# rbuler/multimodal-isic

Measured on AMD Instinct MI355X. Metric: bags/sec (train step) @ 64x224x224 patches/bag, higher is better.
Workload: dtype bf16; 1 GPU; ISIC-shaped attention-MIL: 256 bags x 64x224x224 patches + 128-d radiomics, ResNet-18 encoder, bf16 (BASELINE.json configs[1]); patches_per_bag=64, patch=3x224x224, radiomics_dim=128, parallelism=dp1

## Files before the change

### multimodal-isic_amd/csrc/conv_stem.hip

```cpp
#include <type_traits>

#include "common.h"
#include "slab_sum.inc"
#include "mfma_tile.h"
#include "pool_grad.h"

namespace {

constexpr int TH = 8, TW = 16;
constexpr int PR = 2 * TH + 5, PC = 40;
constexpr int PROW = PC * 8;
constexpr int WROW = 7 * 64 + 16;
constexpr int CPAD = 72;
constexpr int YROW = 128 + 32;
constexpr int STEM_DW_ELEMS = 64 * 7 * 7 * 3;
constexpr int STEM_WGRAD_BLOCKS = 512;
constexpr int STEM_FWD_BLOCKS = 768;

struct StemArgs {
  const unsigned short* in;
  const unsigned short* w;
  unsigned short* out;
  const unsigned short* dy;
  float* dw;
  double* stat_sum;
  double* stat_sumsq;
  int stat_slots;
  int N, Hin, Win, Hout, Wout, tiles_h, tiles_w, total_tiles;
};

constexpr int PATCH_PER_THREAD = (PR * PC + 255) / 256;
__device__ __forceinline__ void fetch_patch(u32x2 (&r)[PATCH_PER_THREAD], const StemArgs& a, int tile, int tid) {
  const int n = tile / (a.tiles_h * a.tiles_w);
  const int t2 = tile - n * (a.tiles_h * a.tiles_w);
  const int oy0 = (t2 / a.tiles_w) * TH, ox0 = (t2 % a.tiles_w) * TW;
#pragma unroll
  for (int u = 0; u < PATCH_PER_THREAD; ++u) {
    const int idx = tid + 256 * u;
    const int pr = idx / PC, pc = idx - pr * PC;
    const int hi = 2 * oy0 - 3 + pr, wi = 2 * ox0 - 3 + pc;
    u32x2 v = {0u, 0u};
    if (tile < a.total_tiles && idx < PR * PC && hi >= 0 && hi < a.Hin && wi >= 0 && wi < a.Win)
      v = *reinterpret_cast<const u32x2*>(a.in + (((size_t)n * a.Hin + hi) * a.Win + wi) * 4);
    r[u] = v;
  }
}
__device__ __forceinline__ void commit_patch(unsigned char* Ps, const u32x2 (&r)[PATCH_PER_THREAD], int tid) {
#pragma unroll
  for (int u = 0; u < PATCH_PER_THREAD; ++u) {
    const int idx = tid + 256 * u;
    if (idx < PR * PC) {
      const int pr = idx / PC, pc = idx - pr * PC;
      *reinterpret_cast<u32x2*>(Ps + pr * PROW + pc * 8) = r[u];
    }
  }
}

__global__ __launch_bounds__(256) void conv_stem_fwd_kernel(StemArgs a) {
  static_assert(TH * TW * CPAD * 2 >= PR * PROW, "the C tile overlays the patch");
  __shared__ __attribute__((aligned(16))) unsigned char smem[64 * WROW + TH * TW * CPAD * 2];
  unsigned char* Ws = smem;
  unsigned char* Ps = smem + 64 * WROW;
  unsigned short* Cs = reinterpret_cast<unsigned short*>(smem + 64 * WROW);
  const int tid = threadIdx.x, lane = tid & 63, wave = tid >> 6;
  const int fi = lane & 15, fg = lane >> 4;

  for (int idx = tid; idx < 64 * 28; idx += 256) {
    const int co = idx / 28, ch = idx - co * 28;
    *reinterpret_cast<u32x4*>(Ws + co * WROW + ch * 16) = *reinterpret_cast<const u32x4*>(a.w + co * 224 + ch * 8);
  }

  u32x2 pre[PATCH_PER_THREAD];
  fetch_patch(pre, a, blockIdx.x, tid);
  float st_s[4][4], st_q[4][4];
#pragma unroll
  for (int j = 0; j < 4; ++j)
#pragma unroll
    for (int r = 0; r < 4; ++r) { st_s[j][r] = 0.f; st_q[j][r] = 0.f; }
  for (int tile = blockIdx.x; tile < a.total_tiles; tile += gridDim.x) {
    const int n = tile / (a.tiles_h * a.tiles_w);
    const int t2 = tile - n * (a.tiles_h * a.tiles_w);
    const int oy0 = (t2 / a.tiles_w) * TH, ox0 = (t2 % a.tiles_w) * TW;
    lds_barrier();
    commit_patch(Ps, pre, tid);
    lds_barrier();
    fetch_patch(pre, a, tile + gridDim.x, tid);

    f32x4 acc[2][4];
#pragma unroll
    for (int i = 0; i < 2; ++i)
#pragma unroll
      for (int j = 0; j < 4; ++j) acc[i][j] = (f32x4){0.f, 0.f, 0.f, 0.f};
#pragma unroll
    for (int kh = 0; kh < 7; ++kh) {
      bf16x8 af[2], bfr[4];
#pragma unroll
      for (int i = 0; i < 2; ++i) {
        const int oyl = wave * 2 + i;
        af[i] = *reinterpret_cast<const bf16x8*>(Ps + (2 * oyl + kh) * PROW + (2 * fi + 2 * fg) * 8);
      }
#pragma unroll
      for (int j = 0; j < 4; ++j)
        bfr[j] = *reinterpret_cast<const bf16x8*>(Ws + (j * 16 + fi) * WROW + kh * 64 + fg * 16);
#pragma unroll
      for (int i = 0; i < 2; ++i)
#pragma unroll
        for (int j = 0; j < 4; ++j)
          acc[i][j] = __builtin_amdgcn_mfma_f32_16x16x32_bf16(bfr[j], af[i], acc[i][j], 0, 0, 0);
    }
    lds_barrier();
#pragma unroll
    for (int i = 0; i < 2; ++i)
#pragma unroll
      for (int j = 0; j < 4; ++j) {
        const int p = (wave * 2 + i) * 16 + fi;
        const u32x2 v = isic_pack_bf16x4(acc[i][j]);
        *reinterpret_cast<u32x2*>(Cs + p * CPAD + j * 16 + fg * 4) = v;
        if (a.stat_sum) {
          const bool in = (oy0 + wave * 2 + i < a.Hout) && (ox0 + fi < a.Wout);
          const float r0 = in ? __uint_as_float(v[0] << 16) : 0.f, r1 = in ? __uint_as_float(v[0] & 0xFFFF0000u) : 0.f;
          const float r2 = in ? __uint_as_float(v[1] << 16) : 0.f, r3 = in ? __uint_as_float(v[1] & 0xFFFF0000u) : 0.f;
          st_s[j][0] += r0; st_q[j][0] += r0 * r0;
          st_s[j][1] += r1; st_q[j][1] += r1 * r1;
          st_s[j][2] += r2; st_q[j][2] += r2 * r2;
          st_s[j][3] += r3; st_q[j][3] += r3 * r3;
        }
      }
    lds_barrier();
    for (int idx = tid; idx < TH * TW * 8; idx += 256) {
      const int p = idx >> 3, ch = idx & 7;
      const int oy = oy0 + (p >> 4), ox = ox0 + (p & 15);
      if (oy < a.Hout && ox < a.Wout)
        __builtin_nontemporal_store(*reinterpret_cast<const u32x4*>(Cs + p * CPAD + ch * 8),
                                    reinterpret_cast<u32x4*>(a.out + (((size_t)n * a.Hout + oy) * a.Wout + ox) * 64 + ch * 8));
    }
  }
  if (a.stat_sum) {
    __shared__ float stat_red[2][4][64];
    lds_barrier();
#pragma unroll
    for (int j = 0; j < 4; ++j)
#pragma unroll
      for (int r = 0; r < 4; ++r) {
        float sv = st_s[j][r], qv = st_q[j][r];
#pragma unroll
        for (int o = 8; o > 0; o >>= 1) { sv += __shfl_xor(sv, o, 16); qv += __shfl_xor(qv, o, 16); }
        if (fi == 0) { stat_red[0][wave][j * 16 + fg * 4 + r] = sv; stat_red[1][wave][j * 16 + fg * 4 + r] = qv; }
      }
    lds_barrier();
    if (tid < 128) {
      const int c = tid & 63, w = tid >> 6;
      const float t = (stat_red[w][0][c] + stat_red[w][1][c]) + (stat_red[w][2][c] + stat_red[w][3][c]);
      const size_t slot = (size_t)(blockIdx.x % a.stat_slots) * 64 + c;
      atomicAdd((w == 0 ? a.stat_sum : a.stat_sumsq) + slot, (double)t);
    }
  }
}

__global__ __launch_bounds__(256) void conv_stem_wgrad_kernel(StemArgs a) {
  __shared__ __attribute__((aligned(16))) unsigned char smem[PR * PROW + TH * TW * YROW];
  unsigned char* Ps = smem;
  unsigned char* Ys = smem + PR * PROW;
  const int tid = threadIdx.x, lane = tid & 63, wave = tid >> 6;
  const int fg = lane >> 4, fi = lane & 15, fq = fi >> 2, fp = fi & 3;
  typedef __attribute__((address_space(3))) s16x4* lds_s16x4;

  f32x4 acc[4][4];
#pragma unroll
  for (int i = 0; i < 4; ++i)
#pragma unroll
    for (int j = 0; j < 4; ++j) acc[i][j] = (f32x4){0.f, 0.f, 0.f, 0.f};

  u32x2 pre[PATCH_PER_THREAD];
  u32x4 prey[4];
  auto fetch_dy = [&](int tile) {
    const int n = tile / (a.tiles_h * a.tiles_w);
    const int t2 = tile - n * (a.tiles_h * a.tiles_w);
    const int oy0 = (t2 / a.tiles_w) * TH, ox0 = (t2 % a.tiles_w) * TW;
#pragma unroll
    for (int u = 0; u < 4; ++u) {
      const int idx = tid + 256 * u;
      const int p = idx >> 3, ch = idx & 7;
      const int oy = oy0 + (p >> 4), ox = ox0 + (p & 15);
      u32x4 v = {0u, 0u, 0u, 0u};
      if (tile < a.total_tiles && oy < a.Hout && ox < a.Wout)
        v = *reinterpret_cast<const u32x4*>(a.dy + (((size_t)n * a.Hout + oy) * a.Wout + ox) * 64 + ch * 8);
      prey[u] = v;
    }
  };
  fetch_patch(pre, a, blockIdx.x, tid);
  fetch_dy(blockIdx.x);
  for (int tile = blockIdx.x; tile < a.total_tiles; tile += gridDim.x) {
    lds_barrier();
    commit_patch(Ps, pre, tid);
#pragma unroll
    for (int u = 0; u < 4; ++u) {
      const int idx = tid + 256 * u;
      *reinterpret_cast<u32x4*>(Ys + (idx >> 3) * YROW + (idx & 7) * 16) = prey[u];
    }
    lds_barrier();
// ... 11 lines not shown
        af[i] = __builtin_bit_cast(bf16x8, t);
      }
#pragma unroll
      for (int j = 0; j < 4; ++j) {
        const int nt = wave + 4 * j;
        const int kh = nt >> 1, half = nt & 1;
        const int khc = kh > 6 ? 6 : kh;
        const unsigned char* p1 = Ps + (2 * (k1 >> 4) + khc) * PROW + (2 * (k1 & 15) + half * 4 + fp) * 8;
        const unsigned char* p2 = Ps + (2 * (k2 >> 4) + khc) * PROW + (2 * (k2 & 15) + half * 4 + fp) * 8;
        const s16x4 lo = __builtin_amdgcn_ds_read_tr16_b64_v4i16((lds_s16x4)p1);
        const s16x4 hi = __builtin_amdgcn_ds_read_tr16_b64_v4i16((lds_s16x4)p2);
        s16x8_t t; t.lo = lo; t.hi = hi;
        bfr[j] = __builtin_bit_cast(bf16x8, t);
      }
#pragma unroll
      for (int i = 0; i < 4; ++i)
#pragma unroll
        for (int j = 0; j < 4; ++j)
          acc[i][j] = __builtin_amdgcn_mfma_f32_16x16x32_bf16(af[i], bfr[j], acc[i][j], 0, 0, 0);
    }
  }
#pragma unroll
  for (int i = 0; i < 4; ++i)
#pragma unroll
    for (int j = 0; j < 4; ++j) {
      const int nt = wave + 4 * j;
      if (nt >= 14) continue;
      const int kh = nt >> 1, kw = (nt & 1) * 4 + (fi >> 2), c = fi & 3;
      if (kw >= 7 || c >= 3) continue;
#pragma unroll
      for (int r = 0; r < 4; ++r) {
        const int co = i * 16 + fg * 4 + r;
        a.dw[(size_t)blockIdx.x * STEM_DW_ELEMS + ((co * 7 + kh) * 7 + kw) * 3 + c] = acc[i][j][r];
      }
    }
}

struct StemBnArgs {
  StemArgs s;
  const unsigned short* y0;
  const unsigned char* argmax;
  const unsigned short* gp;
  const float* mean; const float* rstd; const float* gamma; const float* scale; const float* shift;
  const double* dgamma; const double* dbeta;
  float* dgamma_f32; float* dbeta_f32;
  int Hp, Wp;
};

constexpr int PPIECES = PR * (PROW / 16);
constexpr int PDMA = (PPIECES + 63) / 64;
constexpr int PBUF = PDMA * 1024;
__device__ __attribute__((aligned(256))) unsigned char g_stem_zero_page[256];

struct StemTile { int n, oy0, ox0; };

template <int HALF>
__device__ __forceinline__ void stem_route4_interior(const isic_pool::Windows& w, float (&out)[4][4]) {
  float acc[4][4];
#pragma unroll
  for (int p = 0; p < 4; ++p)
#pragma unroll
    for (int j = 0; j < 4; ++j) acc[p][j] = 0.f;
#pragma unroll
  for (int i = 0; i < 2; ++i)
#pragma unroll
    for (int jw = 0; jw < 2; ++jw) {
      const unsigned lo = w.g[i * 2 + jw][2 * HALF], hi = w.g[i * 2 + jw][2 * HALF + 1];
      const float g[4] = {__uint_as_float(lo << 16), __uint_as_float(lo & 0xFFFF0000u), __uint_as_float(hi << 16),
                          __uint_as_float(hi & 0xFFFF0000u)};
      const unsigned am = w.am[i * 2 + jw][HALF];
#pragma unroll
      for (int dy = i; dy < 2; ++dy)
#pragma unroll
        for (int dx = jw; dx < 2; ++dx) {
          const unsigned code = (unsigned)((dy + 1 - 2 * i) * 3 + (dx + 1 - 2 * jw));
#pragma unroll
          for (int j = 0; j < 4; ++j)
            if (((am >> (j * 8)) & 0xFFu) == code) acc[dy * 2 + dx][j] += g[j];
        }
    }
#pragma unroll
  for (int p = 0; p < 4; ++p)
#pragma unroll
    for (int j = 0; j < 4; ++j) out[p][j] = bf16_bits_to_f32(f32_to_bf16_bits(acc[p][j]));
}

__device__ __forceinline__ float stem_dy_unfused(float kA, float kB, float kD, float y0, float dz) {
#pragma clang fp contract(off)
  const float t = kD + kB * y0;
  return t + kA * dz;
}

template <bool DMA>
__global__ __launch_bounds__(256, 2) void conv_stem_wgrad_bn_kernel(StemBnArgs b) {
  const StemArgs& a = b.s;
  constexpr int PSZ = DMA ? 2 * PBUF : PR * PROW;
  constexpr int PSH = DMA ? 8 : 0;
  __shared__ __attribute__((aligned(16))) unsigned char smem[PSZ + TH * TW * YROW];
  __shared__ __attribute__((aligned(16))) float cst[5][64];
  unsigned char* Ys = smem + PSZ;
  const unsigned lds0 = (unsigned)(size_t)(__attribute__((address_space(3))) unsigned char*)smem;
  const int tid = threadIdx.x, lane = tid & 63, wave = __builtin_amdgcn_readfirstlane(tid >> 6);
  const int fg = lane >> 4, fi = lane & 15, fq = fi >> 2, fp = fi & 3;
  typedef __attribute__((address_space(3))) s16x4* lds_s16x4;
  const unsigned frag_y = (unsigned)((8 * fg + fq) * YROW + 8 * fp);
  const unsigned frag_p = (unsigned)(2 * (fg >> 1) * PROW + (16 * (fg & 1) + 2 * fq + fp) * 8 + PSH);
  const isic_pool::PoolGeom geom{a.Hout, a.Wout, 64, b.Hp, b.Wp};
// ... 199 lines not shown
      if (kw >= 7 || c >= 3) continue;
#pragma unroll
      for (int r = 0; r < 4; ++r) {
        const int co = i * 16 + fg * 4 + r;
        a.dw[(size_t)bid * STEM_DW_ELEMS + ((co * 7 + kh) * 7 + kw) * 3 + c] = acc[i][j][r];
      }
    }
  if (bid == 0 && tid < 64 && b.dgamma_f32) {
    b.dgamma_f32[tid] += (float)b.dgamma[tid];
    b.dbeta_f32[tid] += (float)b.dbeta[tid];
  }
}

__global__ void stem_pack_kernel(const float* __restrict__ w, unsigned short* __restrict__ ws) {
  const int idx = blockIdx.x * blockDim.x + threadIdx.x;
  if (idx >= 64 * 7 * 8 * 4) return;
  const int c = idx & 3, kw = (idx >> 2) & 7, kh = (idx >> 5) % 7, co = idx / 224;
  float v = 0.f;
  if (c < 3 && kw < 7) v = w[((co * 7 + kh) * 7 + kw) * 3 + c];
  ws[idx] = f32_to_bf16_bits(v);
}

int stem_args(StemArgs& a, int N, int Hin, int Win, int Hout, int Wout) {
  if (Hout != (Hin + 6 - 7) / 2 + 1 || Wout != (Win + 6 - 7) / 2 + 1) return ISIC_ERR_BAD_ARG;
  a.N = N; a.Hin = Hin; a.Win = Win; a.Hout = Hout; a.Wout = Wout;
  a.tiles_h = ceil_div(Hout, TH); a.tiles_w = ceil_div(Wout, TW);
  const int64_t tt = (int64_t)N * a.tiles_h * a.tiles_w;
  if (tt > 0x7FFFFFFFLL) return ISIC_ERR_UNSUPPORTED;
  a.total_tiles = (int)tt;
  return ISIC_OK;
}

}

extern "C" {

int isic_conv_stem_fwd_bf16(const uint16_t* in_nhwc4, const uint16_t* w_stem, uint16_t* out, int N, int Hin, int Win,
                            int Hout, int Wout, void* stream) {
  return isic_conv_stem_fwd_stats_bf16(in_nhwc4, w_stem, out, N, Hin, Win, Hout, Wout, nullptr, nullptr, 0, stream);
}

int isic_conv_stem_fwd_stats_bf16(const uint16_t* in_nhwc4, const uint16_t* w_stem, uint16_t* out, int N, int Hin,
                                  int Win, int Hout, int Wout, double* stat_sum, double* stat_sumsq, int stat_slots,
                                  void* stream) {
  ISIC_CHECK_ARG(in_nhwc4 && w_stem && out && N > 0 && Hin > 0 && Win > 0);
  ISIC_CHECK_ARG((stat_sum == nullptr) == (stat_sumsq == nullptr));
  ISIC_CHECK_ARG(!stat_sum || stat_slots > 0);
  StemArgs a;
  a.stat_sum = stat_sum; a.stat_sumsq = stat_sumsq; a.stat_slots = stat_slots > 0 ? stat_slots : 1;
  a.in = in_nhwc4; a.w = w_stem; a.out = out; a.dy = nullptr; a.dw = nullptr;
  int rc = stem_args(a, N, Hin, Win, Hout, Wout);
  if (rc != ISIC_OK) return rc;
  const int grid = a.total_tiles < STEM_FWD_BLOCKS ? a.total_tiles : STEM_FWD_BLOCKS;
  hipLaunchKernelGGL(conv_stem_fwd_kernel, dim3(grid), dim3(256), 0, as_stream(stream), a);
  return isic_launch_status();
}

size_t isic_conv_stem_wgrad_workspace_bytes(void) { return (size_t)STEM_WGRAD_BLOCKS * STEM_DW_ELEMS * sizeof(float); }

int isic_conv_stem_wgrad_bf16(const uint16_t* in_nhwc4, const uint16_t* dy, float* dw, int N, int Hin, int Win,
                              int Hout, int Wout, void* workspace, size_t workspace_bytes, void* stream) {
  ISIC_CHECK_ARG(in_nhwc4 && dy && dw && workspace && N > 0 && Hin > 0 && Win > 0);
  if (workspace_bytes < isic_conv_stem_wgrad_workspace_bytes()) return ISIC_ERR_WORKSPACE;
  StemArgs a;
  a.stat_sum = nullptr; a.stat_sumsq = nullptr; a.stat_slots = 1;
  a.in = in_nhwc4; a.w = nullptr; a.out = nullptr; a.dy = dy; a.dw = reinterpret_cast<float*>(workspace);
  int rc = stem_args(a, N, Hin, Win, Hout, Wout);
  if (rc != ISIC_OK) return rc;
  const int grid = a.total_tiles < STEM_WGRAD_BLOCKS ? a.total_tiles : STEM_WGRAD_BLOCKS;
  hipLaunchKernelGGL(conv_stem_wgrad_kernel, dim3(grid), dim3(256), 0, as_stream(stream), a);
  isic_slab_reduce_launch(ISIC_SLAB_XOR16, reinterpret_cast<const float*>(workspace), grid, STEM_DW_ELEMS, dw, 1.f,
                          as_stream(stream));
  return isic_launch_status();
}

int isic_conv_stem_wgrad_bn_pooled_bf16(const uint16_t* in_nhwc4, const uint16_t* y0, const uint8_t* argmax,
                                        const uint16_t* dy_pooled, const float* mean, const float* rstd,
                                        const float* gamma, const float* scale, const float* shift, const double* dgamma,
                                        const double* dbeta, float* dw, float* dgamma_f32, float* dbeta_f32, int N,
                                        int Hin, int Win, int Hout, int Wout, int Hp, int Wp, void* workspace,
                                        size_t workspace_bytes, void* stream) {
  ISIC_CHECK_ARG(in_nhwc4 && y0 && argmax && dy_pooled && mean && rstd && gamma && scale && shift && dgamma && dbeta && dw);
  ISIC_CHECK_ARG(workspace != nullptr);
  if (workspace_bytes < isic_conv_stem_wgrad_workspace_bytes()) return ISIC_ERR_WORKSPACE;
  ISIC_CHECK_ARG(N > 0 && Hin > 0 && Win > 0 && (dgamma_f32 == nullptr) == (dbeta_f32 == nullptr));
  ISIC_CHECK_ARG(Hp == (Hout + 2 - 3) / 2 + 1 && Wp == (Wout + 2 - 3) / 2 + 1);
  StemBnArgs b;
  StemArgs& a = b.s;
  a.stat_sum = nullptr; a.stat_sumsq = nullptr; a.stat_slots = 1;
  a.in = in_nhwc4; a.w = nullptr; a.out = nullptr; a.dy = nullptr; a.dw = reinterpret_cast<float*>(workspace);
  int rc = stem_args(a, N, Hin, Win, Hout, Wout);
  if (rc != ISIC_OK) return rc;
  b.y0 = y0; b.argmax = argmax; b.gp = dy_pooled; b.mean = mean; b.rstd = rstd; b.gamma = gamma; b.scale = scale;
  b.shift = shift; b.dgamma = dgamma; b.dbeta = dbeta; b.dgamma_f32 = dgamma_f32; b.dbeta_f32 = dbeta_f32;
  b.Hp = Hp; b.Wp = Wp;
  const int grid = a.total_tiles < STEM_WGRAD_BLOCKS ? a.total_tiles : STEM_WGRAD_BLOCKS;
  if (Win % 2 == 0 && (reinterpret_cast<uintptr_t>(in_nhwc4) & 15) == 0)
    hipLaunchKernelGGL(conv_stem_wgrad_bn_kernel<true>, dim3(grid), dim3(256), 0, as_stream(stream), b);
  else
    hipLaunchKernelGGL(conv_stem_wgrad_bn_kernel<false>, dim3(grid), dim3(256), 0, as_stream(stream), b);
  isic_slab_reduce_launch(ISIC_SLAB_XOR16, reinterpret_cast<const float*>(workspace), grid, STEM_DW_ELEMS, dw, 1.f,
                          as_stream(stream));
  return isic_launch_status();
}

int isic_conv_stem_pack_bf16(const float* w_krsc, uint16_t* w_stem, void* stream) {
  ISIC_CHECK_ARG(w_krsc && w_stem);
// ... 6 lines not shown
```

### multimodal-isic_amd/csrc/encoder_ops.hip

```cpp
#include "common.h"
#include "pool_grad.h"

namespace {

using isic_pool::unpack8;
using isic_pool::pack8;
using isic_pool::PoolGeom;

constexpr int FLAT_APPLY = 2, FLAT_BWD = 4;

template <int NACC>
__device__ __forceinline__ void block_reduce_to_global(float (&acc)[NACC][8], int C, double* const (&dst)[NACC]) {
  __shared__ float red[256 * 8];
  const int tid = threadIdx.x, cgs = C >> 3, cg = tid % cgs, rl = tid / cgs, rls = 256 / cgs;
#pragma unroll
  for (int a = 0; a < NACC; ++a) {
    __syncthreads();
#pragma unroll
    for (int j = 0; j < 8; ++j) red[(rl * cgs + cg) * 8 + j] = acc[a][j];
    __syncthreads();
    for (int c = tid; c < C; c += 256) {
      double s = 0.0;
      for (int r = 0; r < rls; ++r) s += (double)red[(r * cgs + (c >> 3)) * 8 + (c & 7)];
      atomicAdd(dst[a] + c, s);
    }
  }
}

__global__ __launch_bounds__(256) void bn_stats_kernel(const unsigned short* __restrict__ x, int64_t rows, int C,
                                                        double* __restrict__ sum, double* __restrict__ sumsq) {
  const int tid = threadIdx.x, cgs = C >> 3, cg = tid % cgs, rl = tid / cgs, rls = 256 / cgs;
  float acc[2][8];
#pragma unroll
  for (int j = 0; j < 8; ++j) { acc[0][j] = 0.f; acc[1][j] = 0.f; }
  const int64_t per_block = ((rows + gridDim.x - 1) / gridDim.x + rls - 1) / rls * rls;
  const int64_t r_end = min(rows, ((int64_t)blockIdx.x + 1) * per_block);
#pragma unroll 4
  for (int64_t r = (int64_t)blockIdx.x * per_block + rl; r < r_end; r += rls) {
    float f[8];
    unpack8(__builtin_nontemporal_load(reinterpret_cast<const u32x4*>(x + r * C + cg * 8)), f);
#pragma unroll
    for (int j = 0; j < 8; ++j) { acc[0][j] += f[j]; acc[1][j] += f[j] * f[j]; }
  }
  double* const dst[2] = {sum, sumsq};
  block_reduce_to_global<2>(acc, C, dst);
}

__global__ __launch_bounds__(256) void bn_finalize_kernel(const double* __restrict__ sum, const double* __restrict__ sumsq,
                                                           int nslots,
                                   int64_t rows, int C, const float* __restrict__ gamma, const float* __restrict__ beta, float eps,
                                   float momentum, float* __restrict__ scale, float* __restrict__ shift,
                                   float* __restrict__ mean_o, float* __restrict__ rstd_o,
                                   float* __restrict__ running_mean, float* __restrict__ running_var) {
// ... 465 lines not shown
      for (int c5 = 0; c5 < 5; ++c5) {
        const int wi = wo0 * 2 - 1 + c5;
        const bool in = hi >= 0 && hi < H && wi >= 0 && wi < W;
        unsigned rb[8];
        float f[8];
#pragma unroll
        for (int q = 0; q < 4; ++q) { rb[2 * q] = raw[kh][c5][q] << 16; rb[2 * q + 1] = raw[kh][c5][q] & 0xFFFF0000u; }
        if (AFFINE) {
#pragma unroll
          for (int j = 0; j < 8; ++j) f[j] = fmaxf(__uint_as_float(rb[j]) * sc[j] + sh[j], 0.f);
          unpack8(pack8(f), f);
        } else {
#pragma unroll
          for (int j = 0; j < 8; ++j) f[j] = __uint_as_float(rb[j]);
        }
        if (in) {
#pragma unroll
          for (int o = 0; o < 2; ++o) {
            const int kw = c5 - 2 * o;
            if (kw < 0 || kw > 2) continue;
            const unsigned code = (unsigned)(kh * 3 + kw);
#pragma unroll
            for (int j = 0; j < 8; ++j) {
              const bool take = f[j] > best[o][j];
              best[o][j] = take ? f[j] : best[o][j];
              pk[o][j] = take ? (rb[j] | code) : pk[o][j];
            }
          }
        }
      }
    }
#pragma unroll
    for (int o = 0; o < 2; ++o) {
      const int wo = wo0 + o;
      if (wo >= Wo) break;
      const int64_t oi = ((((int64_t)n * Ho + ho) * Wo + wo) * cgs + cg);
      __builtin_nontemporal_store(pack8(best[o]), reinterpret_cast<u32x4*>(y + oi * 8));
      if (xsel) {
        u32x4 xs;
#pragma unroll
        for (int q = 0; q < 4; ++q) xs[q] = (pk[o][2 * q] >> 16) | (pk[o][2 * q + 1] & 0xFFFF0000u);
        __builtin_nontemporal_store(xs, reinterpret_cast<u32x4*>(xsel + oi * 8));
      }
      if (argmax) {
        u32x2 p;
        p[0] = (pk[o][0] & 0xFFu) | ((pk[o][1] & 0xFFu) << 8) | ((pk[o][2] & 0xFFu) << 16) | (pk[o][3] << 24);
        p[1] = (pk[o][4] & 0xFFu) | ((pk[o][5] & 0xFFu) << 8) | ((pk[o][6] & 0xFFu) << 16) | (pk[o][7] << 24);
        __builtin_nontemporal_store(p, reinterpret_cast<u32x2*>(argmax + oi * 8));
      }
    }
  }
}

__global__ __launch_bounds__(256) void maxpool_bwd_kernel(const unsigned char* __restrict__ argmax,
                                                           const unsigned short* __restrict__ dy,
                                                           unsigned short* __restrict__ dx, int N, int H, int W, int C,
                                                           int Ho, int Wo) {
  const int cgs = C >> 3;
  const PoolGeom geom{H, W, C, Ho, Wo};
  const int64_t nvec = (int64_t)N * H * W * cgs;
  for (int64_t i = (int64_t)blockIdx.x * blockDim.x + threadIdx.x; i < nvec; i += (int64_t)gridDim.x * blockDim.x) {
    const int cg = (int)(i % cgs);
    int64_t t = i / cgs;
    const int wi = (int)(t % W); t /= W;
    const int hi = (int)(t % H);
    const int n = (int)(t / H);
    float acc[8];
    pooled_grad8(argmax, dy, geom, n, hi, wi, cg, acc);
    *reinterpret_cast<u32x4*>(dx + i * 8) = pack8(acc);
  }
}

__global__ __launch_bounds__(256) void avgpool_fwd_kernel(const unsigned short* __restrict__ x, float* __restrict__ y,
                                                           int HW, int C) {
  __shared__ float part[4][64];
  const int lane = threadIdx.x & 63, wave = threadIdx.x >> 6;
  const int n = blockIdx.x, c = blockIdx.y * 64 + lane;
  float s = 0.f;
  if (c < C)
    for (int p = wave; p < HW; p += 4) s += bf16_bits_to_f32(x[((int64_t)n * HW + p) * C + c]);
  part[wave][lane] = s;
  __syncthreads();
  if (wave == 0 && c < C)
    y[(int64_t)n * C + c] = ((part[0][lane] + part[1][lane]) + (part[2][lane] + part[3][lane])) / (float)HW;
}

__global__ void avgpool_bwd_kernel(const float* __restrict__ dy, unsigned short* __restrict__ dx, int64_t total,
                                   int HW, int C) {
  const float inv = 1.f / (float)HW;
  for (int64_t i = (int64_t)blockIdx.x * blockDim.x + threadIdx.x; i < total; i += (int64_t)gridDim.x * blockDim.x) {
    const int c = (int)(i % C);
    const int64_t n = i / ((int64_t)HW * C);
    dx[i] = f32_to_bf16_bits(dy[n * C + c] * inv);
  }
}

__global__ void add_bf16_kernel(unsigned short* __restrict__ a, const unsigned short* __restrict__ b, int64_t nvec) {
  for (int64_t i = (int64_t)blockIdx.x * blockDim.x + threadIdx.x; i < nvec; i += (int64_t)gridDim.x * blockDim.x) {
    float fa[8], fb[8];
    unpack8(*reinterpret_cast<const u32x4*>(a + i * 8), fa);
    unpack8(*reinterpret_cast<const u32x4*>(b + i * 8), fb);
#pragma unroll
    for (int j = 0; j < 8; ++j) fa[j] += fb[j];
    *reinterpret_cast<u32x4*>(a + i * 8) = pack8(fa);
  }
}
// ... 214 lines not shown
}

int isic_bn_bwd_apply_pair_bf16(const uint16_t* dy, const uint16_t* x, const uint8_t* relu_mask, const float* mean,
                                const float* rstd, const float* gamma, const double* sum_dzx, const double* sum_dz,
                                const uint16_t* x2, const float* mean2, const float* rstd2, const float* gamma2,
                                const double* sum_dzx2, int64_t rows, int C, uint16_t* dx, uint16_t* dx2, float* dgamma_f32,
                                float* dbeta_f32, float* dgamma2_f32, float* dbeta2_f32, void* stream) {
  ISIC_CHECK_ARG(dy && x && relu_mask && mean && rstd && gamma && sum_dzx && sum_dz && x2 && mean2 && rstd2 && gamma2 &&
                 sum_dzx2 && dx && dx2 && rows > 0 && C > 0 && C % 8 == 0);
  ISIC_CHECK_ARG((dgamma_f32 == nullptr) == (dbeta_f32 == nullptr) && (dgamma2_f32 == nullptr) == (dbeta2_f32 == nullptr));
  if (!bn_c_ok(C)) return ISIC_ERR_UNSUPPORTED;
  const int64_t nvec = rows * (C / 8);
  hipLaunchKernelGGL(bn_bwd_apply_pair_kernel, dim3(grid_for(nvec, 256 * FLAT_BWD, STREAM_CAP)), dim3(256), 0,
                     as_stream(stream), dy, x, relu_mask, mean, rstd, gamma, sum_dzx, sum_dz, x2, mean2, rstd2, gamma2, sum_dzx2,
                     rows, C, dx, dx2, dgamma_f32, dbeta_f32, dgamma2_f32, dbeta2_f32);
  return isic_launch_status();
}

int isic_bn_bwd_apply_pooled_bf16(const uint8_t* argmax, const uint16_t* dy_pooled, const uint16_t* x, const float* mean,
                                  const float* rstd, const float* gamma, const double* dgamma, const double* dbeta, int N,
                                  int H, int W, int C, int Ho, int Wo, const float* scale, const float* shift,
                                  uint16_t* dx, float* dgamma_f32, float* dbeta_f32, void* stream) {
  ISIC_CHECK_ARG(argmax && dy_pooled && x && mean && rstd && gamma && dgamma && dbeta && scale && shift && dx);
  ISIC_CHECK_ARG(N > 0 && H > 0 && W > 0 && C > 0 && C % 8 == 0 && Ho == (H + 2 - 3) / 2 + 1 && Wo == (W + 2 - 3) / 2 + 1);
  ISIC_CHECK_ARG((dgamma_f32 == nullptr) == (dbeta_f32 == nullptr));
  if (!bn_c_ok(C)) return ISIC_ERR_UNSUPPORTED;
  const int64_t nvec = (int64_t)N * ((H + 1) / 2) * ((W + 1) / 2) * (C / 8);
  hipLaunchKernelGGL(stem_bn_bwd_apply_kernel, dim3(grid_for(nvec, 256)), dim3(256), 0, as_stream(stream), argmax,
                     dy_pooled, PoolGeom{H, W, C, Ho, Wo}, x, mean, rstd, gamma, dgamma, dbeta, N, scale, shift, dx,
                     dgamma_f32, dbeta_f32);
  return isic_launch_status();
}

int isic_maxpool3x3s2_fwd_bf16(const uint16_t* x, uint16_t* y, uint8_t* argmax, int N, int H, int W, int C, int Ho,
                               int Wo, void* stream) {
  ISIC_CHECK_ARG(x && y && N > 0 && H > 0 && W > 0 && C > 0 && C % 8 == 0);
  ISIC_CHECK_ARG(Ho == (H + 2 - 3) / 2 + 1 && Wo == (W + 2 - 3) / 2 + 1);
  const int64_t nvec = (int64_t)N * Ho * ((Wo + 1) / 2) * (C / 8);
  hipLaunchKernelGGL(maxpool_fwd_kernel<false>, dim3(grid_for(nvec, 256, STREAM_CAP)), dim3(256), 0, as_stream(stream), x, nullptr,
                     nullptr, y, argmax, nullptr, N, H, W, C, Ho, Wo);
  return isic_launch_status();
}

int isic_bn_relu_maxpool3x3s2_fwd_bf16(const uint16_t* x, const float* scale, const float* shift, uint16_t* y,
                                       uint8_t* argmax, int N, int H, int W, int C, int Ho, int Wo, void* stream) {
  return isic_bn_relu_maxpool3x3s2_fwd_sel_bf16(x, scale, shift, y, argmax, nullptr, N, H, W, C, Ho, Wo, stream);
}

int isic_bn_relu_maxpool3x3s2_fwd_sel_bf16(const uint16_t* x, const float* scale, const float* shift, uint16_t* y,
                                           uint8_t* argmax, uint16_t* x_sel, int N, int H, int W, int C, int Ho, int Wo,
                                           void* stream) {
  ISIC_CHECK_ARG(x && scale && shift && y && N > 0 && H > 0 && W > 0 && C > 0 && C % 8 == 0);
  ISIC_CHECK_ARG(Ho == (H + 2 - 3) / 2 + 1 && Wo == (W + 2 - 3) / 2 + 1);
  const int64_t nvec = (int64_t)N * Ho * ((Wo + 1) / 2) * (C / 8);
  hipLaunchKernelGGL(maxpool_fwd_kernel<true>, dim3(grid_for(nvec, 256, STREAM_CAP)), dim3(256), 0, as_stream(stream), x, scale,
                     shift, y, argmax, x_sel, N, H, W, C, Ho, Wo);
  return isic_launch_status();
}

int isic_maxpool3x3s2_bwd_bf16(const uint8_t* argmax, const uint16_t* dy, uint16_t* dx, int N, int H, int W, int C,
                               int Ho, int Wo, void* stream) {
  ISIC_CHECK_ARG(argmax && dy && dx && N > 0 && H > 0 && W > 0 && C > 0 && C % 8 == 0);
  const int64_t nvec = (int64_t)N * H * W * (C / 8);
  hipLaunchKernelGGL(maxpool_bwd_kernel, dim3(grid_for(nvec, 256)), dim3(256), 0, as_stream(stream), argmax, dy, dx, N,
                     H, W, C, Ho, Wo);
  return isic_launch_status();
}

int isic_avgpool_fwd_bf16(const uint16_t* x, float* y, int N, int HW, int C, void* stream) {
  ISIC_CHECK_ARG(x && y && N > 0 && HW > 0 && C > 0);
  hipLaunchKernelGGL(avgpool_fwd_kernel, dim3(N, ceil_div(C, 64)), dim3(256), 0, as_stream(stream), x, y, HW, C);
  return isic_launch_status();
}

int isic_avgpool_bwd_bf16(const float* dy, uint16_t* dx, int N, int HW, int C, void* stream) {
  ISIC_CHECK_ARG(dy && dx && N > 0 && HW > 0 && C > 0);
  const int64_t total = (int64_t)N * HW * C;
  hipLaunchKernelGGL(avgpool_bwd_kernel, dim3(grid_for(total, 256)), dim3(256), 0, as_stream(stream), dy, dx, total, HW,
                     C);
  return isic_launch_status();
}

int isic_add_bf16(uint16_t* a, const uint16_t* b, int64_t n, void* stream) {
  ISIC_CHECK_ARG(a && b && n >= 0 && n % 8 == 0);
  if (n == 0) return ISIC_OK;
  hipLaunchKernelGGL(add_bf16_kernel, dim3(grid_for(n / 8, 256)), dim3(256), 0, as_stream(stream), a, b, n / 8);
  return isic_launch_status();
}

int isic_nchw_to_nhwc4_bf16(const void* in, int in_is_bf16, uint16_t* out, int N, int C, int H, int W, void* stream) {
  ISIC_CHECK_ARG(in && out && N > 0 && C > 0 && C <= 4 && H > 0 && W > 0);
  const int64_t npix = (int64_t)N * H * W;
  const int64_t HW = (int64_t)H * W;
  if (HW % 4 == 0 && HW < (1 << 30) && (reinterpret_cast<uintptr_t>(in) & 15) == 0 && (reinterpret_cast<uintptr_t>(out) & 15) == 0) {
    const dim3 grid((unsigned)((HW / 4 + 255) / 256), (unsigned)(N < 65535 ? N : 65535));
    if (in_is_bf16) hipLaunchKernelGGL(nchw_to_nhwc4_x4_kernel<true>, grid, dim3(256), 0, as_stream(stream), in, out, N, C, (int)HW);
    else hipLaunchKernelGGL(nchw_to_nhwc4_x4_kernel<false>, grid, dim3(256), 0, as_stream(stream), in, out, N, C, (int)HW);
    return isic_launch_status();
  }
  hipLaunchKernelGGL(nchw_to_nhwc4_kernel, dim3(grid_for(npix, 256, STREAM_CAP)), dim3(256), 0, as_stream(stream), in, in_is_bf16,
                     out, npix, C, HW);
  return isic_launch_status();
}

}
```

Before: 950.9 bags/s.

## Write stem conv output directly from registers and add tiled LDS BN-ReLU-maxpool

The stem forward kernel drops its LDS staging of the output tile. It permutes the weight rows so each lane's MFMA accumulators map to contiguous channels, and stores 16-byte pairs straight to global memory. Tile coordinates are advanced incrementally instead of being recomputed with divisions, and a STATS template removes the runtime stats branch. Separately, a new C=64 BN+ReLU+maxpool forward kernel stages an input halo tile into LDS with async global-to-LDS loads, normalizes it once, and computes max/argmax/xsel from LDS, so overlapping 3x3 windows no longer reload from global memory. The risks are more complex index mapping, with possible stat-ordering or argmax code mismatches, and extra LDS use that may lower occupancy.

```diff
diff --git a/multimodal-isic_amd/csrc/conv_stem.hip b/multimodal-isic_amd/csrc/conv_stem.hip
--- a/multimodal-isic_amd/csrc/conv_stem.hip
+++ b/multimodal-isic_amd/csrc/conv_stem.hip
@@ -11,7 +11,6 @@
 constexpr int PR = 2 * TH + 5, PC = 40;
 constexpr int PROW = PC * 8;
 constexpr int WROW = 7 * 64 + 16;
-constexpr int CPAD = 72;
 constexpr int YROW = 128 + 32;
 constexpr int STEM_DW_ELEMS = 64 * 7 * 7 * 3;
 constexpr int STEM_WGRAD_BLOCKS = 512;
@@ -56,35 +55,95 @@
   }
 }
 
-__global__ __launch_bounds__(256) void conv_stem_fwd_kernel(StemArgs a) {
-  static_assert(TH * TW * CPAD * 2 >= PR * PROW, "the C tile overlays the patch");
-  __shared__ __attribute__((aligned(16))) unsigned char smem[64 * WROW + TH * TW * CPAD * 2];
+__device__ __forceinline__ int stem_fwd_lds_row(int co) {
+  return (2 * (co >> 5) + ((co >> 2) & 1)) * 16 + 4 * ((co >> 3) & 3) + (co & 3);
+}
+__device__ __forceinline__ int stem_fwd_channel(int j, int fg, int r) { return 32 * (j >> 1) + 8 * fg + 4 * (j & 1) + r; }
+
+__device__ __forceinline__ void stem_stat4(float* s, float* q, unsigned lo, unsigned hi) {
+#pragma clang fp contract(off)
+  const float r0 = __uint_as_float(lo << 16), r1 = __uint_as_float(lo & 0xFFFF0000u);
+  const float r2 = __uint_as_float(hi << 16), r3 = __uint_as_float(hi & 0xFFFF0000u);
+  s[0] += r0; q[0] += r0 * r0;
+  s[1] += r1; q[1] += r1 * r1;
+  s[2] += r2; q[2] += r2 * r2;
+  s[3] += r3; q[3] += r3 * r3;
+}
+
+struct StemTile { int n, oy0, ox0; };
+
+template <bool STATS>
+__global__ __launch_bounds__(256, 3) void conv_stem_fwd_kernel(StemArgs a) {
+  __shared__ __attribute__((aligned(16))) unsigned char smem[64 * WROW + PR * PROW];
   unsigned char* Ws = smem;
   unsigned char* Ps = smem + 64 * WROW;
-  unsigned short* Cs = reinterpret_cast<unsigned short*>(smem + 64 * WROW);
-  const int tid = threadIdx.x, lane = tid & 63, wave = tid >> 6;
+  const int tid = threadIdx.x, lane = tid & 63, wave = __builtin_amdgcn_readfirstlane(tid >> 6);
   const int fi = lane & 15, fg = lane >> 4;
 
   for (int idx = tid; idx < 64 * 28; idx += 256) {
     const int co = idx / 28, ch = idx - co * 28;
-    *reinterpret_cast<u32x4*>(Ws + co * WROW + ch * 16) = *reinterpret_cast<const u32x4*>(a.w + co * 224 + ch * 8);
-  }
-
+    *reinterpret_cast<u32x4*>(Ws + stem_fwd_lds_row(co) * WROW + ch * 16) =
+        *reinterpret_cast<const u32x4*>(a.w + co * 224 + ch * 8);
+  }
+
+  const int tiles_img = a.tiles_h * a.tiles_w;
+  const int step_n = (int)gridDim.x / tiles_img, step_r = (int)gridDim.x - step_n * tiles_img;
+  const int step_y = (step_r / a.tiles_w) * TH, step_x = (step_r % a.tiles_w) * TW;
+  const int span_y = a.tiles_h * TH, span_x = a.tiles_w * TW;
+  auto advance = [&](StemTile& t) {
+    t.ox0 += step_x;
+    if (t.ox0 >= span_x) { t.ox0 -= span_x; t.oy0 += TH; }
+    t.oy0 += step_y;
+    if (t.oy0 >= span_y) { t.oy0 -= span_y; t.n += 1; }
+    t.n += step_n;
+  };
+  int ppr[PATCH_PER_THREAD], ppc[PATCH_PER_THREAD];
+  unsigned poff[PATCH_PER_THREAD];
+#pragma unroll
+  for (int u = 0; u < PATCH_PER_THREAD; ++u) {
+    const int idx = tid + 256 * u;
+    const bool have = idx < PR * PC;
+    ppr[u] = have ? idx / PC : -(1 << 24);
+    ppc[u] = idx % PC;
+    poff[u] = have ? (unsigned)((ppr[u] * a.Win + ppc[u]) * 8) : 0u;
+  }
   u32x2 pre[PATCH_PER_THREAD];
-  fetch_patch(pre, a, blockIdx.x, tid);
+  auto fetch = [&](const StemTile& t, bool live) {
+    const int hi0 = 2 * t.oy0 - 3, wi0 = 2 * t.ox0 - 3;
+    const unsigned char* org = reinterpret_cast<const unsigned char*>(a.in) + (((int64_t)t.n * a.Hin + hi0) * a.Win + wi0) * 8;
+#pragma unroll
+    for (int u = 0; u < PATCH_PER_THREAD; ++u) {
+      u32x2 v = {0u, 0u};
+      if (live && (unsigned)(hi0 + ppr[u]) < (unsigned)a.Hin && (unsigned)(wi0 + ppc[u]) < (unsigned)a.Win)
+        v = *reinterpret_cast<const u32x2*>(org + poff[u]);
+      pre[u] = v;
+    }
+  };
+
+  StemTile cur;
+  {
+    const int bid = blockIdx.x, t2 = bid % tiles_img;
+    cur.n = bid / tiles_img; cur.oy0 = (t2 / a.tiles_w) * TH; cur.ox0 = (t2 % a.tiles_w) * TW;
+  }
+  fetch(cur, true);
   float st_s[4][4], st_q[4][4];
 #pragma unroll
   for (int j = 0; j < 4; ++j)
 #pragma unroll
     for (int r = 0; r < 4; ++r) { st_s[j][r] = 0.f; st_q[j][r] = 0.f; }
+  const unsigned frag_p = (unsigned)(4 * wave * PROW + (2 * fi + 2 * fg) * 8);
+  const unsigned frag_w = (unsigned)(fi * WROW + fg * 16);
+  const unsigned lane_o = (unsigned)(((fi & ~1) * 64 + 8 * fg + ((fi & 1) ? 32 : 0)) * 2);
+
   for (int tile = blockIdx.x; tile < a.total_tiles; tile += gridDim.x) {
-    const int n = tile / (a.tiles_h * a.tiles_w);
-    const int t2 = tile - n * (a.tiles_h * a.tiles_w);
-    const int oy0 = (t2 / a.tiles_w) * TH, ox0 = (t2 % a.tiles_w) * TW;
+    StemTile nxt = cur;
+    advance(nxt);
     lds_barrier();
-    commit_patch(Ps, pre, tid);
+#pragma unroll
+    for (int u = 0; u < PATCH_PER_THREAD; ++u)
+      if (tid + 256 * u < PR * PC) *reinterpret_cast<u32x2*>(Ps + (tid + 256 * u) * 8) = pre[u];
     lds_barrier();
-    fetch_patch(pre, a, tile + gridDim.x, tid);
+    fetch(nxt, tile + (int)gridDim.x < a.total_tiles);
 
     f32x4 acc[2][4];
 #pragma unroll
@@ -95,49 +154,46 @@
     for (int kh = 0; kh < 7; ++kh) {
       bf16x8 af[2], bfr[4];
 #pragma unroll
+      for (int i = 0; i < 2; ++i) af[i] = *reinterpret_cast<const bf16x8*>(Ps + frag_p + (2 * i + kh) * PROW);
+#pragma unroll
+      for (int j = 0; j < 4; ++j) bfr[j] = *reinterpret_cast<const bf16x8*>(Ws + frag_w + j * 16 * WROW + kh * 64);
+#pragma unroll
+      for (int i = 0; i < 2; ++i)
+#pragma unroll
+        for (int j = 0; j < 4; ++j)
+          acc[i][j] = __builtin_amdgcn_mfma_f32_16x16x32_bf16(bfr[j], af[i], acc[i][j], 0, 0, 0);
+    }
+    const bool full = cur.oy0 + TH <= a.Hout && cur.ox0 + TW <= a.Wout;
+    unsigned char* otile = reinterpret_cast<unsigned char*>(a.out) +
+                           (((int64_t)cur.n * a.Hout + cur.oy0) * a.Wout + cur.ox0) * 128;
+    auto epilogue = [&](auto full_c) {
+      constexpr bool FULL = decltype(full_c)::value;
+#pragma unroll
       for (int i = 0; i < 2; ++i) {
         const int oyl = wave * 2 + i;
-        af[i] = *reinterpret_cast<const bf16x8*>(Ps + (2 * oyl + kh) * PROW + (2 * fi + 2 * fg) * 8);
-      }
-#pragma unroll
-      for (int j = 0; j < 4; ++j)
-        bfr[j] = *reinterpret_cast<const bf16x8*>(Ws + (j * 16 + fi) * WROW + kh * 64 + fg * 16);
-#pragma unroll
-      for (int i = 0; i < 2; ++i)
-#pragma unroll
-        for (int j = 0; j < 4; ++j)
-          acc[i][j] = __builtin_amdgcn_mfma_f32_16x16x32_bf16(bfr[j], af[i], acc[i][j], 0, 0, 0);
-    }
-    lds_barrier();
-#pragma unroll
-    for (int i = 0; i < 2; ++i)
-#pragma unroll
-      for (int j = 0; j < 4; ++j) {
-        const int p = (wave * 2 + i) * 16 + fi;
-        const u32x2 v = isic_pack_bf16x4(acc[i][j]);
-        *reinterpret_cast<u32x2*>(Cs + p * CPAD + j * 16 + fg * 4) = v;
-        if (a.stat_sum) {
-          const bool in = (oy0 + wave * 2 + i < a.Hout) && (ox0 + fi < a.Wout);
-          const float r0 = in ? __uint_as_float(v[0] << 16) : 0.f, r1 = in ? __uint_as_float(v[0] & 0xFFFF0000u) : 0.f;
-          const float r2 = in ? __uint_as_float(v[1] << 16) : 0.f, r3 = in ? __uint_as_float(v[1] & 0xFFFF0000u) : 0.f;
-          st_s[j][0] += r0; st_q[j][0] += r0 * r0;
-          st_s[j][1] += r1; st_q[j][1] += r1 * r1;
-          st_s[j][2] += r2; st_q[j][2] += r2 * r2;
-          st_s[j][3] += r3; st_q[j][3] += r3 * r3;
+        const bool in = FULL || ((cur.oy0 + oyl < a.Hout) && (cur.ox0 + fi < a.Wout));
+        u32x4 vv[2];
+#pragma unroll
+        for (int j = 0; j < 4; ++j) {
+          const unsigned w0 = isic_pack_bf16x2(acc[i][j][0], acc[i][j][1]), w1 = isic_pack_bf16x2(acc[i][j][2], acc[i][j][3]);
+          vv[j >> 1][2 * (j & 1)] = w0;
+          vv[j >> 1][2 * (j & 1) + 1] = w1;
+          if (STATS) stem_stat4(st_s[j], st_q[j], in ? w0 : 0u, in ? w1 : 0u);
         }
-      }
-    lds_barrier();
-    for (int idx = tid; idx < TH * TW * 8; idx += 256) {
-      const int p = idx >> 3, ch = idx & 7;
-      const int oy = oy0 + (p >> 4), ox = ox0 + (p & 15);
-      if (oy < a.Hout && ox < a.Wout)
-        __builtin_nontemporal_store(*reinterpret_cast<const u32x4*>(Cs + p * CPAD + ch * 8),
-                                    reinterpret_cast<u32x4*>(a.out + (((size_t)n * a.Hout + oy) * a.Wout + ox) * 64 + ch * 8));
-    }
-  }
-  if (a.stat_sum) {
+        u32x4 da, db;
+        isic_pair_rows(vv[0], vv[1], fi & 1, da, db);
+        unsigned char* o = otile + (int64_t)oyl * a.Wout * 128 + lane_o;
+        const bool row = FULL || cur.oy0 + oyl < a.Hout;
+        if (row && (FULL || cur.ox0 + (fi & ~1) < a.Wout)) __builtin_nontemporal_store(da, reinterpret_cast<u32x4*>(o));
+        if (row && (FULL || cur.ox0 + (fi | 1) < a.Wout)) __builtin_nontemporal_store(db, reinterpret_cast<u32x4*>(o + 128));
+      }
+    };
+    if (full) epilogue(std::true_type{});
+    else epilogue(std::false_type{});
+    cur = nxt;
+  }
+  if (STATS) {
     __shared__ float stat_red[2][4][64];
-    lds_barrier();
 #pragma unroll
     for (int j = 0; j < 4; ++j)
 #pragma unroll
@@ -145,7 +201,8 @@
         float sv = st_s[j][r], qv = st_q[j][r];
 #pragma unroll
         for (int o = 8; o > 0; o >>= 1) { sv += __shfl_xor(sv, o, 16); qv += __shfl_xor(qv, o, 16); }
-        if (fi == 0) { stat_red[0][wave][j * 16 + fg * 4 + r] = sv; stat_red[1][wave][j * 16 + fg * 4 + r] = qv; }
+        const int c = stem_fwd_channel(j, fg, r);
+        if (fi == 0) { stat_red[0][wave][c] = sv; stat_red[1][wave][c] = qv; }
       }
     lds_barrier();
     if (tid < 128) {
@@ -263,7 +320,6 @@
 constexpr int PBUF = PDMA * 1024;
 __device__ __attribute__((aligned(256))) unsigned char g_stem_zero_page[256];
 
-struct StemTile { int n, oy0, ox0; };
 
 template <int HALF>
 __device__ __forceinline__ void stem_route4_interior(const isic_pool::Windows& w, float (&out)[4][4]) {
@@ -569,7 +625,8 @@
   int rc = stem_args(a, N, Hin, Win, Hout, Wout);
   if (rc != ISIC_OK) return rc;
   const int grid = a.total_tiles < STEM_FWD_BLOCKS ? a.total_tiles : STEM_FWD_BLOCKS;
-  hipLaunchKernelGGL(conv_stem_fwd_kernel, dim3(grid), dim3(256), 0, as_stream(stream), a);
+  if (stat_sum) hipLaunchKernelGGL(conv_stem_fwd_kernel<true>, dim3(grid), dim3(256), 0, as_stream(stream), a);
+  else hipLaunchKernelGGL(conv_stem_fwd_kernel<false>, dim3(grid), dim3(256), 0, as_stream(stream), a);
   return isic_launch_status();
 }
 
diff --git a/multimodal-isic_amd/csrc/encoder_ops.hip b/multimodal-isic_amd/csrc/encoder_ops.hip
--- a/multimodal-isic_amd/csrc/encoder_ops.hip
+++ b/multimodal-isic_amd/csrc/encoder_ops.hip
@@ -1,4 +1,5 @@
 #include "common.h"
+#include "mfma_tile.h"
 #include "pool_grad.h"
 
 namespace {
@@ -570,6 +571,145 @@
   }
 }
 
+template <int TPH, int TPW>
+struct PoolTile {
+  static constexpr int PRH = 2 * TPH + 1, PCW = 2 * TPW + 1;
+  static constexpr int NT = TPH * TPW * 4;
+  static constexpr int NW = NT / 64;
+  static constexpr int NPIECE = PRH * PCW * 8;
+  static constexpr int NINS = (NPIECE + 63) / 64;
+  static constexpr int RAWB = NINS * 1024;
+  static_assert(NT % 64 == 0 && TPW % 2 == 0, "whole waves, whole output pairs");
+  static_assert((NINS + NW - 1) / NW <= 32, "one validity bit per piece of a thread");
+};
+
+template <int TPH, int TPW>
+__global__ __launch_bounds__(TPH * TPW * 4) void bn_relu_maxpool_c64_kernel(
+    const unsigned short* __restrict__ x, const float* __restrict__ scale, const float* __restrict__ shift,
+    unsigned short* __restrict__ y, unsigned char* __restrict__ argmax, unsigned short* __restrict__ xsel, int H, int W,
+    int Ho, int Wo, int tiles_h, int tiles_w) {
+  using T = PoolTile<TPH, TPW>;
+  __shared__ __attribute__((aligned(16))) unsigned char smem[T::RAWB + T::NPIECE * 16];
+  const unsigned lds0 = (unsigned)(size_t)(__attribute__((address_space(3))) unsigned char*)smem;
+  const unsigned char* raw = smem;
+  unsigned char* nrm = smem + T::RAWB;
+  const int tid = threadIdx.x, lane = tid & 63, wave = __builtin_amdgcn_readfirstlane(tid >> 6);
+  const int tile = blockIdx.x;
+  const int tw = tile % tiles_w, t1 = tile / tiles_w, th = t1 % tiles_h, n = t1 / tiles_h;
+  const int ho0 = th * TPH, wo0 = tw * TPW, hi0 = 2 * ho0 - 1, wi0 = 2 * wo0 - 1;
+
+  constexpr int NU = (T::NINS + T::NW - 1) / T::NW;
+  constexpr int STEP = T::NT / 8, STEP_R = STEP / T::PCW, STEP_C = STEP % T::PCW;
+  const int cg = tid & 7;
+  const unsigned char* img = reinterpret_cast<const unsigned char*>(x) + (int64_t)n * H * W * 128;
+  unsigned okmask = 0;
+  {
+    int pr = (tid >> 3) / T::PCW, pc = (tid >> 3) - pr * T::PCW;
+#pragma unroll
+    for (int u = 0; u < NU; ++u) {
+      const int hi = hi0 + pr, wi = wi0 + pc;
+      if (pr < T::PRH && (unsigned)hi < (unsigned)H && (unsigned)wi < (unsigned)W) okmask |= 1u << u;
+      if (wave + T::NW * u < T::NINS) {
+        const int hc = min(max(hi, 0), H - 1), wc = min(max(wi, 0), W - 1);
+        isic_glds16_s(img, (unsigned)((hc * W + wc) * 128 + cg * 16),
+                      __builtin_amdgcn_readfirstlane(lds0 + (unsigned)((wave + T::NW * u) * 1024)));
+      }
+      pr += STEP_R; pc += STEP_C;
+      if (pc >= T::PCW) { pc -= T::PCW; pr += 1; }
+    }
+  }
+  float sc[8], sh[8];
+#pragma unroll
+  for (int j = 0; j < 8; ++j) { sc[j] = scale[cg * 8 + j]; sh[j] = shift[cg * 8 + j]; }
+  asm volatile("s_waitcnt vmcnt(0)" ::: "memory");
+
+#pragma unroll
+  for (int u = 0; u < NU; ++u) {
+    const int q = tid + T::NT * u;
+    if (q < T::NPIECE) {
+      const bool ok = (okmask >> u) & 1u;
+      const u32x4 r = *reinterpret_cast<const u32x4*>(raw + q * 16);
+      u32x4 o;
+#pragma unroll
+      for (int i = 0; i < 4; ++i) {
+        const float lo = fmaxf(fmaf(__uint_as_float(r[i] << 16), sc[2 * i], sh[2 * i]), 0.f);
+        const float hi = fmaxf(fmaf(__uint_as_float(r[i] & 0xFFFF0000u), sc[2 * i + 1], sh[2 * i + 1]), 0.f);
+        o[i] = ok ? isic_pack_bf16x2(lo, hi) : 0x80008000u;
+      }
+      *reinterpret_cast<u32x4*>(nrm + q * 16) = o;
+    }
+  }
+  lds_barrier();
+
+  const int tp = tid >> 3, oh = tp / (TPW / 2), pw = tp - oh * (TPW / 2);
+  const int ho = ho0 + oh, wq = wo0 + 2 * pw;
+  const unsigned base = (unsigned)(((2 * oh) * T::PCW + 4 * pw) * 128 + cg * 16);
+  int best[2][8];
+#pragma unroll
+  for (int o = 0; o < 2; ++o)
+#pragma unroll
+    for (int j = 0; j < 8; ++j) best[o][j] = (int)0x80000000u;
+#pragma unroll
+  for (int kh = 0; kh < 3; ++kh)
+#pragma unroll
+    for (int c5 = 0; c5 < 5; ++c5) {
+      const u32x4 v = *reinterpret_cast<const u32x4*>(nrm + base + (kh * T::PCW + c5) * 128);
+#pragma unroll
+      for (int o = 0; o < 2; ++o) {
+        const int kw = c5 - 2 * o;
+        if (kw < 0 || kw > 2) continue;
+        const unsigned K = 8u - (unsigned)(kh * 3 + kw);
+#pragma unroll
+        for (int i = 0; i < 4; ++i) {
+          best[o][2 * i] = max(best[o][2 * i], (int)((v[i] << 16) | K));
+          best[o][2 * i + 1] = max(best[o][2 * i + 1], (int)((v[i] & 0xFFFF0000u) | K));
+        }
+      }
+    }
+#pragma unroll
+  for (int o = 0; o < 2; ++o) {
+    const int wo = wq + o;
+    if (ho >= Ho || wo >= Wo) continue;
+    const int64_t oi = (((int64_t)n * Ho + ho) * Wo + wo) * 8 + cg;
+    u32x4 yv;
+#pragma unroll
+    for (int i = 0; i < 4; ++i) yv[i] = ((unsigned)best[o][2 * i] >> 16) | ((unsigned)best[o][2 * i + 1] & 0xFFFF0000u);
+    __builtin_nontemporal_store(yv, reinterpret_cast<u32x4*>(y + oi * 8));
+    unsigned code[8];
+#pragma unroll
+    for (int j = 0; j < 8; ++j) code[j] = 8u - ((unsigned)best[o][j] & 0xFu);
+    if (xsel) {
+      unsigned rv[8];
+#pragma unroll
+      for (int j = 0; j < 8; ++j) {
+        const unsigned kh = (code[j] * 11u) >> 5;
+        rv[j] = *reinterpret_cast<const unsigned short*>(raw + base + o * 256 + kh * ((T::PCW - 3) * 128) + code[j] * 128 + j * 2);
+      }
+      u32x4 xs;
+#pragma unroll
+      for (int i = 0; i < 4; ++i) xs[i] = rv[2 * i] | (rv[2 * i + 1] << 16);
+      __builtin_nontemporal_store(xs, reinterpret_cast<u32x4*>(xsel + oi * 8));
+    }
+    if (argmax) {
+      u32x2 p;
+      p[0] = code[0] | (code[1] << 8) | (code[2] << 16) | (code[3] << 24);
+      p[1] = code[4] | (code[5] << 8) | (code[6] << 16) | (code[7] << 24);
+      __builtin_nontemporal_store(p, reinterpret_cast<u32x2*>(argmax + oi * 8));
+    }
+  }
+}
+
+template <int TPH, int TPW>
+bool launch_bn_relu_maxpool_c64(const uint16_t* x, const float* scale, const float* shift, uint16_t* y, uint8_t* argmax,
+                                uint16_t* x_sel, int N, int H, int W, int Ho, int Wo, hipStream_t stream) {
+  const int tiles_h = ceil_div(Ho, TPH), tiles_w = ceil_div(Wo, TPW);
+  const int64_t tiles = (int64_t)N * tiles_h * tiles_w;
+  if (tiles > 0x7FFFFFFFLL || (int64_t)H * W > (1 << 24)) return false;
+  hipLaunchKernelGGL((bn_relu_maxpool_c64_kernel<TPH, TPW>), dim3((unsigned)tiles), dim3(PoolTile<TPH, TPW>::NT), 0, stream, x,
+                     scale, shift, y, argmax, x_sel, H, W, Ho, Wo, tiles_h, tiles_w);
+  return true;
+}
+
 __global__ __launch_bounds__(256) void maxpool_bwd_kernel(const unsigned char* __restrict__ argmax,
                                                            const unsigned short* __restrict__ dy,
                                                            unsigned short* __restrict__ dx, int N, int H, int W, int C,
@@ -890,6 +1030,9 @@
                                            void* stream) {
   ISIC_CHECK_ARG(x && scale && shift && y && N > 0 && H > 0 && W > 0 && C > 0 && C % 8 == 0);
   ISIC_CHECK_ARG(Ho == (H + 2 - 3) / 2 + 1 && Wo == (W + 2 - 3) / 2 + 1);
+  if (C == 64 && (reinterpret_cast<uintptr_t>(x) & 15) == 0 &&
+      launch_bn_relu_maxpool_c64<8, 8>(x, scale, shift, y, argmax, x_sel, N, H, W, Ho, Wo, as_stream(stream)))
+    return isic_launch_status();
   const int64_t nvec = (int64_t)N * Ho * ((Wo + 1) / 2) * (C / 8);
   hipLaunchKernelGGL(maxpool_fwd_kernel<true>, dim3(grid_for(nvec, 256, STREAM_CAP)), dim3(256), 0, as_stream(stream), x, scale,
                      shift, y, argmax, x_sel, N, H, W, C, Ho, Wo);
```

Result: faster. 960.7 bags/s (median of 6 runs) (+1.0%).
